# fabrii4/AutoEncoder-FFT

Measured on AMD Instinct MI355X. Metric: frames/s fwd+bwd (FFT mode, 512x512, 4 layers), higher is better.
Workload: dtype f32; 1 GPU; cfg3-P2: 512x512x3 frames, 4 pairs 3->8->16->32->64, 5x5, pool 2/layer, FFT mode, fwd + 1 loop-body iteration per pair (operator form); every step produces reconstructions, batch-mean gradients, updated weights and the per-pair post-update MSE partial sums -- the sums themselves are formed by the next step's gradient launch (no per-step MSE read-back inside the timed loop); frames_per_gpu=32, global_batch=32, parallelism=dp1

## Files before the change

### autoencoder-fft_amd/csrc/internal.h

```cpp
#pragma once
#include <hip/hip_runtime.h>
#include <stddef.h>
#include <stdint.h>

namespace aefft {

extern unsigned dev_flags;
inline bool flag(unsigned f) { return (dev_flags & f) != 0; }

constexpr int TW_N = 4096;
hipError_t upload_twiddles(hipStream_t st);
bool fft_size_supported(int n);

hipError_t launch_r2c(const void* in, float2* out, float2* mid, long planes, int Nx, int Ny,
                      int Nxs, int Nys, hipStream_t st, hipEvent_t done = nullptr , bool in_u8 = false);
constexpr int OPIN_COLS = 4;
constexpr int OPMSE_PACKED_STEPS = 16;
constexpr int CH_MAXSTEPS = 40;
constexpr int CH_VMAX = 128;
struct OpIn { const float2* A; const float2* Xf; int D0, Nx0, Ny0; };
hipError_t launch_c2r(const float2* in, void* out, float2* mid, long planes, int Nxi, int Nyi,
                      int Nx, int Ny, float scale, hipStream_t st, const OpIn* opin = nullptr, bool out_u8 = false);
size_t fft_mid_elems(long planes, int Nx, int Wc);
bool fft_size_supported_any(int n);
size_t fft_any_ws_elems(long planes, int Nx, int Ny);
hipError_t launch_r2c_any(const float* in, float2* out, float2* w1, float2* w2, long planes, int Nx, int Ny, hipStream_t st);
hipError_t launch_c2r_any(const float2* in, float* out, float2* w1, float2* w2, long planes, int Nx, int Ny, float scale, hipStream_t st);
bool fft_size_mixed(int n);
bool fft_size_smooth(int n);
hipError_t fft_mixed_prepare(int n);
hipError_t launch_mix_r2c_rows(const void* in, float2* mid, long npairs, int Ny, int Wc, hipStream_t st, bool in_u8);
hipError_t launch_mix_fwd_cols(const float2* mid, float2* out, long planes, int Nx, int Wc, int Nxs, hipStream_t st, hipEvent_t done);
hipError_t launch_mix_inv_cols(const float2* in, float2* mid, long planes, int Nx, int Wc, int Nxi, hipStream_t st,
                               const OpIn* opin = nullptr );
hipError_t launch_mix_c2r_rows(const float2* mid, void* out, long npairs, int Ny, int Wc, float scale, hipStream_t st, bool out_u8 = false);

struct Contract {
    const float2* A; long a_r, a_k;
    const float2* A2;
    const float2* B; long b_k, b_c;
    float2* Out;     long o_r, o_c;
    int R, C, K;
    long P;
    bool conjA, conjB;
    float preDivB;
    float postDiv;
    const float* bias; float biasScale;
    bool biasAfterFirst;
    int biasColP1;
    int upNx, upNy, upNxs, upNys;
    float2* Out2; int dnNx, dnNy, dnNxs, dnNys;
// ... 183 lines not shown
```

### autoencoder-fft_amd/csrc/opform_kernels.hip

```cpp
#include "../../include/aefft.h"
#include "internal.h"
#include <hip/hip_ext.h>
#include "device_util.h"
#include "opform_device.h"
#include <algorithm>
#include <type_traits>

namespace aefft {

__device__ __forceinline__ float2 cmul(float2 a, float2 b) { return make_float2(a.x * b.x - a.y * b.y, a.x * b.y + a.y * b.x); }
__device__ __forceinline__ float2 cmulc(float2 a, float2 b) { return make_float2(a.x * b.x + a.y * b.y, a.y * b.x - a.x * b.y); }
__device__ __forceinline__ void cfma2(float2& acc, float2 a, float2 b) { acc.x = fmaf(a.x, b.x, acc.x); acc.x = fmaf(-a.y, b.y, acc.x); acc.y = fmaf(a.x, b.y, acc.y); acc.y = fmaf(a.y, b.x, acc.y); }
__device__ __forceinline__ void cfmac(float2& acc, float2 a, float2 b) { acc.x = fmaf(a.x, b.x, acc.x); acc.x = fmaf(a.y, b.y, acc.x); acc.y = fmaf(a.y, b.x, acc.y); acc.y = fmaf(-a.x, b.y, acc.y); }
__device__ __forceinline__ float2 ld8(const float2* base, unsigned e) { return *reinterpret_cast<const float2*>(reinterpret_cast<const char*>(base) + e * 8u); }
__device__ __forceinline__ void st8(float2* base, unsigned e, float2 v) { *reinterpret_cast<float2*>(reinterpret_cast<char*>(base) + e * 8u) = v; }

template <typename MG> __device__ __forceinline__ float quad_centred(const float2 (&r)[OPC], MG Mget)
{
    float2 r3 = r[OPC - 1];
#pragma unroll
    for (int j = 0; j < OPC - 1; ++j) cfma2(r3, r[j], Mget(j * OPC + OPC - 1));
    float part = Mget(OPC * OPC - 1).x * (r3.x * r3.x + r3.y * r3.y);
#pragma unroll
    for (int k = 0; k < OPC - 1; ++k) {
// ... 631 lines not shown
#pragma unroll
    for (int off = 32; off > 0; off >>= 1) part += __shfl_down(part, off, 64);
    float* red = reinterpret_cast<float*>(Ts + (size_t)DM * OPC * BT);
    if ((threadIdx.x & 63) == 0) red[threadIdx.x >> 6] = part;
    __syncthreads();
    if (threadIdx.x == 0) {
        const float tot = (red[0] + red[1]) + (red[2] + red[3]);
        if (tot != 0.f) atomicAdd(q.slots + (blockIdx.x % MSE_SLOTS) * MSE_SLOT_STRIDE, tot * q.scale);
    }
}

#ifndef AEFFT_X_CHAINPIPE
#define AEFFT_X_CHAINPIPE 1
#endif
#ifndef AEFFT_X_CH_DEPTH
#define AEFFT_X_CH_DEPTH 4
#endif
#ifndef AEFFT_X_CH_PK
#define AEFFT_X_CH_PK 1
#endif
__device__ __forceinline__ void cfma_pk(float2& acc, float2 a, float2 b)
{
#if AEFFT_X_CH_PK
    typedef float v2f __attribute__((ext_vector_type(2)));
    v2f r = {acc.x, acc.y};
    const v2f av = {a.x, a.y}, bv = {b.x, b.y};
    asm("v_pk_fma_f32 %0, %1, %2, %0 op_sel:[0,0,0] op_sel_hi:[0,1,1]" : "+v"(r) : "v"(av), "v"(bv));
    asm("v_pk_fma_f32 %0, %1, %2, %0 op_sel:[1,1,0] op_sel_hi:[1,0,1] neg_lo:[0,1,0]" : "+v"(r) : "v"(av), "v"(bv));
    acc = make_float2(r.x, r.y);
#else
    cfma2(acc, a, b);
#endif
}
constexpr int CH_NE = 4, CH_DEPTH = AEFFT_X_CH_DEPTH, CH_NB = CH_DEPTH + 1, CH_KSH_MAX = 4, CH_BLOCK = 12;
template <int N> __device__ __forceinline__ float dpp_row_shl(float v)
{
    return __builtin_bit_cast(float, __builtin_amdgcn_update_dpp(0, __builtin_bit_cast(int, v), 0x100 + N, 0xf, 0xf, true));
}
struct ChainSrc {
    const ChainArgs& g;
    __device__ __forceinline__ unsigned off(int i) const { return g.st_off[i]; }
    __device__ __forceinline__ unsigned desc(int i) const { return g.st_desc[i]; }
    __device__ __forceinline__ const float* bias(unsigned lv, bool enc) const { return enc ? g.lv[lv].b : g.lv[lv].p; }
    __device__ __forceinline__ float NN(unsigned lv) const { return (float)g.lv[lv].Nx * (float)g.lv[lv].Ny; }
    __device__ __forceinline__ float2* out(unsigned lv) const { return g.lv[lv].O; }
    __device__ __forceinline__ unsigned Pc() const { return (unsigned)g.Pc; }
};
template <class SRC>
__device__ __forceinline__ void chain_step_load(const SRC& g, const float2* __restrict__ rec, const int i, float2 (&w)[CH_NE], float& bv)
{
    const unsigned d = g.desc(i), off = g.off(i) & 0xffffffu;
    const unsigned R = d & 255u, K = (d >> 8) & 255u, k0 = (d >> 16) & 127u, ksh = (d >> 23) & 7u;
    const unsigned tid = threadIdx.x;
    const unsigned r = min(tid >> ksh, R - 1u), ks = tid & ((1u << ksh) - 1u);
    const unsigned row = off + r * K, e0 = row + k0 + ks, elast = row + K - 1u;
#pragma unroll
    for (int u = 0; u < CH_NE; ++u) w[u] = ld8(rec, min(e0 + ((unsigned)u << ksh), elast));
    bv = g.bias(d >> 29, (d >> 28) & 1u)[r];
}
template <bool DUAL, class SRC>
__device__ __forceinline__ void chain_step_compute(const SRC& g, const int i, const float2 (&w)[CH_NE], const float bv, float2 (&acc)[OPC], float2 (&acc2)[OPC],
                                                   float2* const Wl, const int t)
{
    static_assert(OPC == 4, "two 16-byte LDS accesses per row of V");
    const unsigned d = g.desc(i), par = g.off(i) >> 31;
    const bool dual = DUAL && ((g.off(i) >> 30) & 1u);
    const unsigned R = d & 255u, K = (d >> 8) & 255u, k0 = (d >> 16) & 127u, ksh = (d >> 23) & 7u;
// ... 84 lines not shown
            }
        }
    }
    __syncthreads();
#if defined(AEFFT_X_WGTIME) && AEFFT_X_WGTIME
    if (threadIdx.x == 0) reinterpret_cast<unsigned long long*>(Wl + 5 * CH_VMAX * OPC + 4 + OPC * OPC)[(enc ? lv : 7 - lv) & 7] = wall_clock64();
#endif
}
template <int I, bool DUAL, class SRC>
__device__ __forceinline__ void chain_steps(const SRC& g, const float2* __restrict__ rec, const int base, const int nb, float2 (&w)[CH_NB][CH_NE], float (&bv)[CH_NB],
                                            float2 (&acc)[OPC], float2 (&acc2)[OPC], float2* const Wl, const int t)
{
    if constexpr (I < CH_BLOCK) {
        if (I >= nb) return;
        chain_step_load(g, rec, base + min(I + CH_DEPTH, nb - 1), w[(I + CH_DEPTH) % CH_NB], bv[(I + CH_DEPTH) % CH_NB]);
        chain_step_compute<DUAL>(g, base + I, w[I % CH_NB], bv[I % CH_NB], acc, acc2, Wl, t);
        chain_steps<I + 1, DUAL, SRC>(g, rec, base, nb, w, bv, acc, acc2, Wl, t);
    }
}
template <bool DUAL, class SRC, class INIT>
__device__ __forceinline__ void chain_run_steps(const SRC& g, const float2* __restrict__ rec, const int n, float2* const Wl, const int t, INIT init)
{
    float2 w[CH_NB][CH_NE];
    float bv[CH_NB];
    float2 acc[OPC], acc2[OPC];
    for (int base = 0; base < n; base += CH_BLOCK) {
        const int nb = min(n - base, CH_BLOCK);
#pragma unroll
        for (int j = 0; j < CH_DEPTH; ++j) chain_step_load(g, rec, base + min(j, nb - 1), w[j], bv[j]);
        if (base == 0) { init(); __syncthreads(); }
        chain_steps<0, DUAL, SRC>(g, rec, base, nb, w, bv, acc, acc2, Wl, t);
    }
}
static bool chain_add_stage(unsigned* st_off, unsigned* st_desc, int* n, int cap, int R, int K, unsigned off, int par, bool enc, int lvl)
{
    int ksh = 0;
    while (ksh < CH_KSH_MAX && (2 << ksh) * R <= 256 && (1 << ksh) < K) ++ksh;
    const int kc = CH_NE << ksh;
    for (int k0 = 0; k0 < K; k0 += kc) {
        if (*n >= cap || off >= (1u << 24) || k0 > 127 || R > 255 || K > 255) return false;
        st_off[*n] = off | ((unsigned)(par & 1) << 31);
        st_desc[*n] = (unsigned)R | ((unsigned)K << 8) | ((unsigned)k0 << 16) | ((unsigned)ksh << 23) | ((k0 + kc >= K ? 1u : 0u) << 26) |
                      ((k0 == 0 ? 1u : 0u) << 27) | ((enc ? 1u : 0u) << 28) | ((unsigned)lvl << 29);
        ++*n;
    }
    return true;
}

constexpr size_t OPMSE_PACKED_LDS = sizeof(float2) * (3 * CH_VMAX * OPC + 2 + OPC * OPC) + 128;
struct PackedMseSrc {
    const OpMseGroup& g; const OpMsePair& q;
    __device__ __forceinline__ unsigned off(int i) const { return g.pst_off[i]; }
    __device__ __forceinline__ unsigned desc(int i) const { return g.pst_desc[i]; }
    __device__ __forceinline__ const float* bias(unsigned, bool enc) const { return enc ? q.b : q.p; }
    __device__ __forceinline__ float NN(unsigned) const { return (float)q.Nx * (float)q.Ny; }
    __device__ __forceinline__ float2* out(unsigned) const { return nullptr; }
    __device__ __forceinline__ unsigned Pc() const { return 0u; }
};
__device__ __forceinline__ void opmse_packed(const OpMseGroup& g, int p, long t, float2* sh)
{
    float2 *Va = sh + 2 * CH_VMAX * OPC;
    float* redp = reinterpret_cast<float*>(sh + 3 * CH_VMAX * OPC);
    const OpMsePair q = g.q[p];
    const int dD = q.dD, dM = q.dM;
    const float2* rec = g.Wp + t * g.E;
    const float2* Vc;
    float2* Ms = sh + 3 * CH_VMAX * OPC + 2;
    const long um = map_up(t, q.Nx, q.Ny, g.Nx0, g.Ny0);
    if (g.pst_n > 0) {
        const PackedMseSrc src{g, q};
        chain_run_steps<false>(src, rec, g.pst_n, sh, (int)t, [&]() {
            float2 mv = make_float2(0.f, 0.f);
            if (threadIdx.x < OPC * OPC) mv = g.Mhat[(long)threadIdx.x * g.P0 + um];
            for (int i = threadIdx.x; i < dD * OPC; i += 256) { const int a = i / OPC, k = i - a * OPC; const float2 v = q.A[((long)k * dD + a) * q.P + t]; sh[i] = v; Va[i] = v; }
            if (threadIdx.x < OPC * OPC) Ms[threadIdx.x] = mv;
        });
        Vc = sh;
    } else {
        float2 *Vb = sh, *Vd = sh + CH_VMAX * OPC;
        if (threadIdx.x < OPC * OPC) Ms[threadIdx.x] = g.Mhat[(long)threadIdx.x * g.P0 + um];
        for (int i = threadIdx.x; i < dD * OPC; i += 256) { const int a = i / OPC, k = i - a * OPC; Va[i] = q.A[((long)k * dD + a) * q.P + t]; }
        const float NN = (float)q.Nx * (float)q.Ny;
        __syncthreads();
        chain_stage_rec(rec + g.offC, Va, Vb, dM, dD, 1.0f / (float)dM, q.b, NN, t == 0, nullptr, 0, 0);
        __syncthreads();
        chain_stage_rec(rec + g.offF, Vb, Vd, dD, dM, 1.0f / (float)dD, q.p, NN, t == 0, nullptr, 0, 0);
        __syncthreads();
        Vc = Vd;
    }
    float part = 0.f;
    if ((int)threadIdx.x < dD) {
        const int a = threadIdx.x;
        float2 r[OPC];
#pragma unroll
        for (int k = 0; k < OPC; ++k) { const float2 av = Va[a * OPC + k], fv = Vc[a * OPC + k]; r[k] = make_float2(av.x - fv.x, av.y - fv.y); }
        part = quad_centred(r, [&](int e) { return Ms[e]; });
        const int nyr = q.Ny / 2 + 1;
        const int j = (int)((unsigned)t % (unsigned)nyr);
        part *= (j > 0 && j < nyr - 1) ? 2.f : 1.f;
    }
#pragma unroll
    for (int off = 32; off > 0; off >>= 1) part += __shfl_down(part, off, 64);
    if ((threadIdx.x & 63) == 0) redp[threadIdx.x >> 6] = part;
    __syncthreads();
    if (threadIdx.x == 0) {
        const float tot = (redp[0] + redp[1]) + (redp[2] + redp[3]);
        if (tot != 0.f) atomicAdd(q.slots + (blockIdx.x % MSE_SLOTS) * MSE_SLOT_STRIDE, tot * q.scale);
    }
}

template <bool LEAN>
__device__ __forceinline__ void opmse_dispatch(const OpMseGroup& g, float2* sh)
{
    const int blk = (int)blockIdx.x - g.base;
    int p = g.n - 1;
#pragma unroll
    for (int i = 6; i >= 0; --i) if (i < g.n - 1 && blk >= g.start[i] - g.base) p = i;
    if (p == g.n - 1 && g.Wp) { opmse_packed(g, p, (long)blockIdx.x - g.start[p], sh); return; }
    if (LEAN || g.q[p].G) { opmse_gbody(g, p, sh); return; }
    if constexpr (!LEAN) {
        const int bt = g.bt[p];
        if (bt == 32) opmse_small_body<8>(g, p, sh);
        else if (bt == 16) opmse_body<16>(g, p, sh);
        else if (bt == 8) opmse_body<8>(g, p, sh);
        else opmse_body<4>(g, p, sh);
    }
}

static hipError_t opmse_geometry(OpMseGroup& g, int base, long* nblocks, size_t* lds_out, bool fused = false )
{
    if (g.n < 1 || g.n > 8) return hipErrorInvalidValue;
    long total = base;
    size_t lds = 0;
    g.base = base;
    for (int i = g.n - 1; i >= 0; --i) {
        const OpMsePair& q = g.q[i];
        int bt = 16;
        while (bt > 4 && ((q.P + bt - 1) / bt < 128 || (size_t)OPC * (q.dD + q.dM) * bt * sizeof(float2) > 48 * 1024)) bt >>= 1;
        size_t need = (size_t)OPC * (q.dD + q.dM) * bt * sizeof(float2) + 64 + (size_t)256 * OPC * sizeof(float2) + (size_t)OPC * OPC * bt * sizeof(float2);
        const bool pk = i == g.n - 1 && g.Wp && q.dD <= CH_VMAX && q.dM <= CH_VMAX;
        if (pk) {
            need = OPMSE_PACKED_LDS;
            int n = 0;
            const bool fits = chain_add_stage(g.pst_off, g.pst_desc, &n, OPMSE_PACKED_STEPS, q.dM, q.dD, (unsigned)g.offC, 0, true, 0) &&
                              chain_add_stage(g.pst_off, g.pst_desc, &n, OPMSE_PACKED_STEPS, q.dD, q.dM, (unsigned)g.offF, 1, false, 0);
            g.pst_n = fits && AEFFT_X_CHAINPIPE ? n : 0;
        }
        else if (q.G) {
            if ((double)q.dD * q.dD * q.P * 8.0 >= 4294967296.0) return hipErrorInvalidValue;
            bt = msgrad_bt(q.dD, q.P);
            need = sizeof(float2) * ((size_t)OPC * q.dD * bt + (size_t)OPC * OPC * bt) + 64;
        } else if (q.dM == 8 && q.dD <= 4 && !flag(AEFFT_F_NOFAST)) { bt = 32; need = (size_t)OPC * (4 + 8) * 32 * sizeof(float2) + 64; }
        if (i == g.n - 1 && !pk) g.Wp = nullptr;
        if (need > 150 * 1024) return hipErrorInvalidValue;
        g.bt[i] = bt;
        lds = std::max(lds, need);
        g.start[i] = (int)total;
        total += pk ? (fused ? 0 : q.P) : (q.P + bt - 1) / bt;
    }
    if (total >= (1L << 31)) return hipErrorInvalidValue;
    g.start[g.n] = (int)total;
    *nblocks = total - base; *lds_out = lds;
    return hipSuccess;
}

}

namespace aefft {

template <int NK> __global__ __launch_bounds__(256) void kspec_packed_kernel(const PackArgs g)
{
    extern __shared__ float2 pk_lds[];
    kspec_packed_body<NK>(g, PackPhasePow2{}, blockIdx.x, blockIdx.y, pk_lds);
}
template <int NK> __global__ __launch_bounds__(256) void kspec_packed_mod_kernel(const PackArgs g, const PackTabs t)
{
    extern __shared__ float2 pk_lds[];
    kspec_packed_body<NK>(g, PackPhaseMod{t}, blockIdx.x, blockIdx.y, pk_lds);
}

void pack_blocks(PackArgs& g)
{
    int nb = 0;
    for (int i = 0; i < g.nseg; ++i)
        for (int l0 = 0; l0 < g.seg[i].n && nb < 128; l0 += 256) { g.blk_seg[nb] = (unsigned char)i; g.blk_start[nb] = l0; ++nb; }
    g.nblk = nb;
}

hipError_t launch_kspec_packed(PackArgs& g, hipStream_t st)
{
    if (g.nseg < 1 || g.nseg > 16 || g.L < 1 || g.L > 8 || g.E < 1 || (g.Nk != 3 && g.Nk != 5)) return hipErrorInvalidValue;
    pack_blocks(g);
    const dim3 grid((unsigned)g.nblk, (unsigned)pack_yblocks(g));
    if (pack_mod(g)) {
        PackTabs t{};
        const hipError_t e = pack_tabs(g, t);
        if (e != hipSuccess) return e;
        if (g.Nk == 3) kspec_packed_mod_kernel<3><<<grid, 256, kspec_packed_lds(3), st>>>(g, t);
        else kspec_packed_mod_kernel<5><<<grid, 256, kspec_packed_lds(5), st>>>(g, t);
        return hipGetLastError();
    }
    if (g.Nk == 3) kspec_packed_kernel<3><<<grid, 256, kspec_packed_lds(3), st>>>(g);
    else kspec_packed_kernel<5><<<grid, 256, kspec_packed_lds(5), st>>>(g);
    return hipGetLastError();
}

template <bool DUAL>
__device__ __forceinline__ void chain_item_run(const ChainArgs& g, const int t, float2* Wl, const OpMseGroup* mse)
{
    const ChainSrc src{g};
    constexpr int VS = CH_VMAX * OPC;
    float2* Ms = Wl + 5 * VS;
    chain_run_steps<DUAL>(src, g.Wp + (long)t * g.E, g.st_n, Wl, t, [&]() {
        float2 mv = make_float2(0.f, 0.f);
        if (DUAL) {
            const OpMsePair& q = mse->q[mse->n - 1];
            if (threadIdx.x < OPC * OPC) mv = mse->Mhat[(long)threadIdx.x * mse->P0 + map_up(t, q.Nx, q.Ny, mse->Nx0, mse->Ny0)];
            const int dD = q.dD;
            for (int i = threadIdx.x; i < dD * OPC; i += 256) { const int a = i / OPC, k = i - a * OPC; Wl[2 * VS + i] = q.A[((long)k * dD + a) * q.P + t]; }
        }
        for (int i = threadIdx.x; i < VS; i += 256) { const int k = i / OPC, c = i - k * OPC; Wl[i] = make_float2((k == c && c < OPC - 1) ? 1.f : 0.f, 0.f); }
        if (DUAL && threadIdx.x < OPC * OPC) Ms[threadIdx.x] = mv;
    });
    if (DUAL) {
        const OpMsePair& q = mse->q[mse->n - 1];
        const float2 *Va = Wl + 2 * VS, *Vc = Wl + 4 * VS;
        float* redp = reinterpret_cast<float*>(Ms + OPC * OPC);
        float part = 0.f;
        if ((int)threadIdx.x < q.dD) {
            const int a = threadIdx.x;
            float2 r[OPC];
#pragma unroll
            for (int k = 0; k < OPC; ++k) { const float2 av = Va[a * OPC + k], fv = Vc[a * OPC + k]; r[k] = make_float2(av.x - fv.x, av.y - fv.y); }
            part = quad_centred(r, [&](int e) { return Ms[e]; });
            const int nyr = q.Ny / 2 + 1;
            const int j = (int)((unsigned)t % (unsigned)nyr);
            part *= (j > 0 && j < nyr - 1) ? 2.f : 1.f;
        }
#pragma unroll
        for (int off = 32; off > 0; off >>= 1) part += __shfl_down(part, off, 64);
        if ((threadIdx.x & 63) == 0) redp[threadIdx.x >> 6] = part;
        __syncthreads();
        if (threadIdx.x == 0) {
            const float tot = (redp[0] + redp[1]) + (redp[2] + redp[3]);
            if (tot != 0.f) atomicAdd(q.slots + (blockIdx.x % MSE_SLOTS) * MSE_SLOT_STRIDE, tot * q.scale);
        }
    }
#if defined(AEFFT_X_WGTIME) && AEFFT_X_WGTIME
    if (threadIdx.x == 0 && g_wgtime && blockIdx.x < WGT_MAX)
        for (int k = 0; k < 8; ++k) g_wgtime[(size_t)5 * WGT_MAX * 2 + ((size_t)4 * WGT_MAX + blockIdx.x) * 8 + k] = reinterpret_cast<unsigned long long*>(Wl + 5 * CH_VMAX * OPC + 4 + OPC * OPC)[k];
#endif
}

#if defined(AEFFT_X_WGTIME) && AEFFT_X_WGTIME
constexpr int CH_ITEM_VECS = 5;
#else
constexpr int CH_ITEM_VECS = 2;
#endif
constexpr int CH_BT = 8;
template <bool FUSE>
__device__ __forceinline__ void chain_body(const ChainArgs& g, const int bx, float2* Wl, const OpMseGroup* mse = nullptr)
{
    const int tid = threadIdx.x;
    const int L = g.L;
    if (AEFFT_X_CHAINPIPE && (long)bx < g.Pc && g.st_n > 0) { chain_item_run<FUSE>(g, bx, Wl, mse); return; }
    if ((long)bx < g.Pc) {
        const int t = bx;
        const bool dc = t == 0;
        const float2* rec = g.Wp + (long)t * g.E;
        for (int i = tid; i < CH_VMAX * OPC; i += 256) { const int k = i / OPC, c = i - k * OPC; Wl[i] = make_float2((k == c && c < OPC - 1) ? 1.f : 0.f, 0.f); }
        int off = 0, si = 0;
        auto run = [&](int R, int K, float scale, const float* bias, float NN, float2* out) {
            __syncthreads();
            AEFFT_WGSTAMP(4, si & 7);
            chain_stage_rec(rec + off, Wl + (si & 1) * (CH_VMAX * OPC), Wl + ((si + 1) & 1) * (CH_VMAX * OPC), R, K, scale, bias, NN, dc, out, g.Pc, t);
            off += (R * K + 1) & ~1; ++si;
        };
        for (int j = 1; j < L; ++j) { const ChainLevel& w = g.lv[j - 1]; run(w.dM, w.dD, 1.0f / (float)w.dM, w.b, (float)w.Nx * (float)w.Ny, nullptr); }
        { const ChainLevel& w = g.lv[L - 1]; run(w.dM, w.dD, 1.0f / (float)w.dM, w.b, (float)w.Nx * (float)w.Ny, nullptr); }
        for (int j = L - 1; j >= 0; --j) { const ChainLevel& v = g.lv[j]; run(v.dD, v.dM, 1.0f / (float)v.dD, v.p, (float)v.Nx * (float)v.Ny, v.O); }
        return;
    }
    int j = 1;
#pragma unroll
    for (int i = 2; i < 8; ++i) if (i < L && bx >= g.tile_start[i]) j = i;
    const int bt = g.tile_bt[j], RT = 256 / bt;
    const int bl = tid & (bt - 1), ry = tid / bt;
    const ChainLevel lj = g.lv[j];
    const long s0 = (long)(bx - g.tile_start[j]) * bt;
    const long s = min(s0 + bl, lj.P - 1);
    const bool ok = s0 + bl < lj.P;
    for (int i = tid; i < OPC * OPC * bt; i += 256) { const int c = (i / bt) % OPC, k = i / (bt * OPC); Wl[i] = make_float2((k == c && c < OPC - 1) ? 1.f : 0.f, 0.f); }
#pragma unroll 1
    for (int i = 1; i <= j; ++i) {
        const ChainLevel& w = g.lv[i - 1];
        const long sbi = i == j ? s : map_up(s, lj.Nx, lj.Ny, g.lv[i].Nx, g.lv[i].Ny);
        const long sbm = map_up(s, lj.Nx, lj.Ny, w.Nx, w.Ny);
        const int R = w.dM, K = w.dD;
// ... 5 lines not shown
            float2 acc[OPC];
#pragma unroll
            for (int c = 0; c < OPC; ++c) acc[c] = make_float2(0.f, 0.f);
            const long pst = w.Cc ? g.lv[i].P : w.P;
            const float2* Wp = (w.Cc ? w.Cc + sbi : w.C + sbm) + (long)r * K * pst;
            auto grp = [&](int k0, auto NU) {
                constexpr int U = decltype(NU)::value;
                float2 wv[U];
#pragma unroll
                for (int u = 0; u < U; ++u) wv[u] = Wp[(long)(k0 + u) * pst];
#pragma unroll
                for (int u = 0; u < U; ++u)
#pragma unroll
                    for (int c = 0; c < OPC; ++c) cfma2(acc[c], wv[u], Vin[((k0 + u) * OPC + c) * bt + bl]);
            };
            int k0 = 0;
            for (; k0 + 16 <= K; k0 += 16) grp(k0, std::integral_constant<int, 16>{});
            if (k0 + 8 <= K) { grp(k0, std::integral_constant<int, 8>{}); k0 += 8; }
            if (k0 + 4 <= K) { grp(k0, std::integral_constant<int, 4>{}); k0 += 4; }
            if (k0 + 2 <= K) { grp(k0, std::integral_constant<int, 2>{}); k0 += 2; }
            if (k0 < K) grp(k0, std::integral_constant<int, 1>{});
#pragma unroll
            for (int c = 0; c < OPC; ++c) { acc[c].x *= scale; acc[c].y *= scale; }
            if (sbi == 0) acc[OPC - 1].x += w.b[r] * NN;
#pragma unroll
            for (int c = 0; c < OPC; ++c) {
                Vout[(r * OPC + c) * bt + bl] = acc[c];
                if (i == j && ok) lj.A[((long)c * R + r) * lj.P + s] = acc[c];
            }
        }
    }
}

__global__ __launch_bounds__(256) void chain_kernel(const ChainArgs g)
{
    extern __shared__ float2 Wl[];
    chain_body<false>(g, blockIdx.x, Wl);
}

static hipError_t chain_geometry(ChainArgs& g, long* nblocks, size_t* lds_out, bool* fuse = nullptr, unsigned offC = 0, unsigned offF = 0)
{
    if (g.L < 1 || g.L > 8 || !g.Wp || g.Pc < 1) return hipErrorInvalidValue;
    for (int l = 0; l < g.L; ++l) {
        if (g.lv[l].dD > CH_VMAX || g.lv[l].dM > CH_VMAX) return hipErrorInvalidValue;
        if (l + 1 < g.L && (size_t)2 * g.lv[l].dM * OPC * CH_BT > CH_WL) return hipErrorInvalidValue;
    }
    {
        int n = 0; unsigned off = 0;
        bool fits = true, offs_ok = true;
        int dual_lo = 0, dual_hi = 0;
        for (int si = 0; si < 2 * g.L && fits; ++si) {
            const bool enc = si < g.L;
            const int l = enc ? si : 2 * g.L - 1 - si;
            const int R = enc ? g.lv[l].dM : g.lv[l].dD, K = enc ? g.lv[l].dD : g.lv[l].dM;
            if (si == g.L - 1) { dual_lo = n; offs_ok = offs_ok && off == offC; }
            if (si == g.L) offs_ok = offs_ok && off == offF;
            fits = chain_add_stage(g.st_off, g.st_desc, &n, CH_MAXSTEPS, R, K, off, si & 1, enc, l);
            if (si == g.L) dual_hi = n;
            off += (unsigned)((R * K + 1) & ~1);
        }
        g.st_n = fits ? n : 0;
        if (fuse) {
            *fuse = *fuse && fits && offs_ok && AEFFT_X_CHAINPIPE;
            if (*fuse) for (int i = dual_lo; i < dual_hi; ++i) g.st_off[i] |= 1u << 30;
        }
        if ((double)OPC * CH_VMAX * (double)g.Pc * sizeof(float2) >= 4294967296.0) return hipErrorInvalidValue;
    }
    long total = g.Pc;
    int vt = OPC * OPC * 32;
    for (int j = 1; j < g.L; ++j) {
        int rj = OPC;
        for (int l = 0; l < j; ++l) rj = std::max(rj, g.lv[l].dM);
        int bt = 32;
        while (bt > CH_BT && bt * rj > 256) bt >>= 1;
        g.tile_bt[j] = bt;
        vt = std::max(vt, rj * OPC * bt);
        g.tile_start[j] = (int)total; total += (g.lv[j].P + bt - 1) / bt;
    }
    g.tile_start[g.L] = (int)total;
    if (total >= (1L << 31)) return hipErrorInvalidValue;
    g.vt_elems = vt;
    *nblocks = total;
    *lds_out = std::max(sizeof(float2) * 2 * g.vt_elems, sizeof(float2) * ((fuse && *fuse ? 5 : CH_ITEM_VECS) * (size_t)CH_VMAX * OPC + OPC * OPC + 4) + 256 );
    return hipSuccess;
}

hipError_t launch_chain(ChainArgs& g, hipStream_t st, hipEvent_t done)
{
    long total; size_t lds;
    const hipError_t eg = chain_geometry(g, &total, &lds);
    if (eg != hipSuccess) return eg;
    if (done) hipExtLaunchKernelGGL(chain_kernel, dim3((unsigned)total), dim3(256), lds, st, nullptr, done, 0, g);
    else chain_kernel<<<dim3((unsigned)total), 256, lds, st>>>(g);
    return hipGetLastError();
}

#ifndef AEFFT_X_TAIL_W
#define AEFFT_X_TAIL_W 6
#endif
#ifndef AEFFT_X_TAIL_WF
#define AEFFT_X_TAIL_WF 5
#endif
template <bool LEAN, bool FUSE>
__global__ __launch_bounds__(256, LEAN ? (FUSE ? AEFFT_X_TAIL_WF : AEFFT_X_TAIL_W) : 4) void tail_kernel(const OpMseGroup g, const ChainArgs ch, const UpdateGroup ug, const int nchain, const int nupd_start)
{
    AEFFT_WGTIME(4);
    extern __shared__ float2 sh[];
    if ((int)blockIdx.x < nchain) { chain_body<FUSE>(ch, blockIdx.x, sh, &g); return; }
    if ((int)blockIdx.x >= nupd_start) {
        const int blk = blockIdx.x - nupd_start;
        int p = 0;
#pragma unroll
        for (int i = 1; i < 8; ++i) if (i < ug.n && blk >= ug.start[i]) p = i;
        update_weights_part(ug.a[p], blk - ug.start[p]);
        return;
    }
    opmse_dispatch<LEAN>(g, sh);
}

static UpdateGroup g_tail_ug_none{};
static ChainArgs g_tail_chain_none{};
hipError_t launch_opmse_group(OpMseGroup& g, hipStream_t st, ChainArgs* chain, const UpdateGroup* weights_upd)
{
    long nchain = 0, nmse = 0;
    size_t lds_c = 0, lds_m = 0;
#ifndef AEFFT_X_FUSEMSE
#define AEFFT_X_FUSEMSE 1
#endif
    bool fuse = AEFFT_X_FUSEMSE && chain && g.Wp && chain->Wp == g.Wp && chain->E == g.E && chain->Pc == g.q[g.n - 1].P &&
                g.q[g.n - 1].dD <= CH_VMAX && g.q[g.n - 1].dM <= CH_VMAX && g.q[g.n - 1].dD <= 256;
    if (chain) { const hipError_t e = chain_geometry(*chain, &nchain, &lds_c, &fuse, (unsigned)g.offC, (unsigned)g.offF); if (e != hipSuccess) return e; }
    { const hipError_t e = opmse_geometry(g, (int)nchain, &nmse, &lds_m, false); if (e != hipSuccess) return e; }
    if (fuse && nchain + nmse < 4 * 1536 && !flag(AEFFT_F_CHAINMSE)) {
        fuse = false;
        for (int i = 0; i < chain->st_n; ++i) chain->st_off[i] &= ~(1u << 30);
        const hipError_t e = chain_geometry(*chain, &nchain, &lds_c); if (e != hipSuccess) return e;
    }
    if (fuse) {
        const hipError_t e = opmse_geometry(g, (int)nchain, &nmse, &lds_m, true); if (e != hipSuccess) return e;
        if (!g.Wp) return hipErrorInvalidValue;
    }
    int nupd = 0;
    UpdateGroup ug = g_tail_ug_none;
    if (weights_upd && weights_upd->n > 0) {
        ug = *weights_upd;
        for (int i = 0; i < ug.n; ++i) { ug.start[i] = nupd; nupd += (ug.a[i].dM * ug.a[i].dD * ug.a[i].Nk * ug.a[i].Nl + 255) / 256; }
        ug.start[ug.n] = nupd;
    }
    const size_t lds = std::max(lds_c, lds_m);
#ifndef AEFFT_X_LEANTAIL
#define AEFFT_X_LEANTAIL 1
#endif
    bool lean = AEFFT_X_LEANTAIL != 0;
    for (int i = 0; i < g.n && lean; ++i) lean = g.q[i].G != nullptr || (i == g.n - 1 && g.Wp != nullptr);
    const long total = nchain + nmse + nupd;
    if (total >= (1L << 31)) return hipErrorInvalidValue;
    auto go = [&](auto LEANT, auto FUSET) -> hipError_t {
        constexpr bool LN = decltype(LEANT)::value, FS = decltype(FUSET)::value;
        if (lds > 64 * 1024) {
            const hipError_t e = hipFuncSetAttribute(reinterpret_cast<const void*>(tail_kernel<LN, FS>), hipFuncAttributeMaxDynamicSharedMemorySize, (int)lds);
            if (e != hipSuccess) return e;
        }
        tail_kernel<LN, FS><<<dim3((unsigned)total), 256, lds, st>>>(g, chain ? *chain : g_tail_chain_none, ug, (int)nchain, (int)(nchain + nmse));
        return hipGetLastError();
    };
    if (lean) return fuse ? go(std::true_type{}, std::true_type{}) : go(std::true_type{}, std::false_type{});
    return fuse ? go(std::false_type{}, std::true_type{}) : go(std::false_type{}, std::false_type{});
}

}

#if defined(AEFFT_X_WGTIME) && AEFFT_X_WGTIME
extern "C" int aefft_debug_wgtime_opform(void* p) { return aefft::wgtime_set_tu(p); }
#endif
```

Before: 222,400 frames/s.

## Specialize chain step pipeline at compile time for known layer plans

Result: no change. 223,500 frames/s (median of 5 runs) (+0.5%).

```diff
diff --git a/autoencoder-fft_amd/csrc/chain_plan.h b/autoencoder-fft_amd/csrc/chain_plan.h
--- /dev/null
+++ b/autoencoder-fft_amd/csrc/chain_plan.h
@@ -0,0 +1,91 @@
+#pragma once
+
+namespace aefft {
+
+constexpr int OPMSE_PACKED_STEPS = 16;
+constexpr int CH_MAXSTEPS = 40;
+constexpr int CH_NE = 4, CH_KSH_MAX = 4;
+
+constexpr unsigned CH_OFF_DUAL = 1u << 30;
+constexpr bool chain_add_stage(unsigned* st_off, unsigned* st_desc, int* n, int cap, int R, int K, unsigned off, int par, bool enc, int lvl)
+{
+    int ksh = 0;
+    while (ksh < CH_KSH_MAX && (2 << ksh) * R <= 256 && (1 << ksh) < K) ++ksh;
+    const int kc = CH_NE << ksh;
+    for (int k0 = 0; k0 < K; k0 += kc) {
+        if (*n >= cap || off >= (1u << 24) || k0 > 127 || R > 255 || K > 255) return false;
+        st_off[*n] = off | ((unsigned)(par & 1) << 31);
+        st_desc[*n] = (unsigned)R | ((unsigned)K << 8) | ((unsigned)k0 << 16) | ((unsigned)ksh << 23) | ((k0 + kc >= K ? 1u : 0u) << 26) |
+                      ((k0 == 0 ? 1u : 0u) << 27) | ((enc ? 1u : 0u) << 28) | ((unsigned)lvl << 29);
+        ++*n;
+    }
+    return true;
+}
+
+constexpr bool chain_list_build(unsigned* st_off, unsigned* st_desc, int* n_out, int L, const int* dD, const int* dM, int* dual_lo, int* dual_hi,
+                                unsigned* recC, unsigned* recF)
+{
+    int n = 0; unsigned off = 0;
+    bool fits = true;
+    for (int si = 0; si < 2 * L && fits; ++si) {
+        const bool enc = si < L;
+        const int l = enc ? si : 2 * L - 1 - si;
+        const int R = enc ? dM[l] : dD[l], K = enc ? dD[l] : dM[l];
+        if (si == L - 1) { *dual_lo = n; *recC = off; }
+        if (si == L) *recF = off;
+        fits = chain_add_stage(st_off, st_desc, &n, CH_MAXSTEPS, R, K, off, si & 1, enc, l);
+        if (si == L) *dual_hi = n;
+        off += (unsigned)((R * K + 1) & ~1);
+    }
+    *n_out = n;
+    return fits;
+}
+constexpr bool chain_list_build_mse(unsigned* st_off, unsigned* st_desc, int* n_out, int dD, int dM, unsigned offC, unsigned offF)
+{
+    int n = 0;
+    const bool fits = chain_add_stage(st_off, st_desc, &n, OPMSE_PACKED_STEPS, dM, dD, offC, 0, true, 0) &&
+                      chain_add_stage(st_off, st_desc, &n, OPMSE_PACKED_STEPS, dD, dM, offF, 1, false, 0);
+    *n_out = n;
+    return fits;
+}
+
+struct ChainPlan {
+    unsigned off[CH_MAXSTEPS] = {}, desc[CH_MAXSTEPS] = {}; int n = 0;
+    unsigned moff[OPMSE_PACKED_STEPS] = {}, mdesc[OPMSE_PACKED_STEPS] = {}; int mn = 0;
+};
+constexpr int CH_PLAN_MIN = 3, CH_PLAN_MAX = 5;
+constexpr ChainPlan chain_plan_make(int PL)
+{
+    ChainPlan p;
+    int dD[8] = {}, dM[8] = {};
+    for (int l = 0; l < PL; ++l) { dM[l] = 8 << l; dD[l] = l ? dM[l - 1] : 3; }
+    int lo = 0, hi = 0; unsigned recC = 0, recF = 0;
+    if (!chain_list_build(p.off, p.desc, &p.n, PL, dD, dM, &lo, &hi, &recC, &recF)) p.n = 0;
+    for (int i = lo; i < hi && i < p.n; ++i) p.off[i] |= CH_OFF_DUAL;
+    if (!chain_list_build_mse(p.moff, p.mdesc, &p.mn, dD[PL - 1], dM[PL - 1], recC, recF)) p.mn = 0;
+    return p;
+}
+template <int PL> inline constexpr ChainPlan chain_plan_v = chain_plan_make(PL);
+
+constexpr bool chain_list_same(const unsigned* off, const unsigned* desc, int n, const unsigned* poff, const unsigned* pdesc, int pn)
+{
+    if (n != pn || n < 1) return false;
+    for (int i = 0; i < n; ++i) if (((off[i] ^ poff[i]) & ~CH_OFF_DUAL) != 0 || desc[i] != pdesc[i]) return false;
+    return true;
+}
+constexpr int chain_plan_of(const unsigned* off, const unsigned* desc, int n)
+{
+    if (chain_list_same(off, desc, n, chain_plan_v<3>.off, chain_plan_v<3>.desc, chain_plan_v<3>.n)) return 3;
+    if (chain_list_same(off, desc, n, chain_plan_v<4>.off, chain_plan_v<4>.desc, chain_plan_v<4>.n)) return 4;
+    if (chain_list_same(off, desc, n, chain_plan_v<5>.off, chain_plan_v<5>.desc, chain_plan_v<5>.n)) return 5;
+    return 0;
+}
+constexpr int chain_plan_of_mse(const unsigned* off, const unsigned* desc, int n)
+{
+    if (chain_list_same(off, desc, n, chain_plan_v<3>.moff, chain_plan_v<3>.mdesc, chain_plan_v<3>.mn)) return 3;
+    if (chain_list_same(off, desc, n, chain_plan_v<4>.moff, chain_plan_v<4>.mdesc, chain_plan_v<4>.mn)) return 4;
+    if (chain_list_same(off, desc, n, chain_plan_v<5>.moff, chain_plan_v<5>.mdesc, chain_plan_v<5>.mn)) return 5;
+    return 0;
+}
+
+}
diff --git a/autoencoder-fft_amd/csrc/internal.h b/autoencoder-fft_amd/csrc/internal.h
--- a/autoencoder-fft_amd/csrc/internal.h
+++ b/autoencoder-fft_amd/csrc/internal.h
@@ -2,6 +2,7 @@
 #include <hip/hip_runtime.h>
 #include <stddef.h>
 #include <stdint.h>
+#include "chain_plan.h"
 
 namespace aefft {
 
@@ -15,8 +16,6 @@
 hipError_t launch_r2c(const void* in, float2* out, float2* mid, long planes, int Nx, int Ny,
                       int Nxs, int Nys, hipStream_t st, hipEvent_t done = nullptr , bool in_u8 = false);
 constexpr int OPIN_COLS = 4;
-constexpr int OPMSE_PACKED_STEPS = 16;
-constexpr int CH_MAXSTEPS = 40;
 constexpr int CH_VMAX = 128;
 struct OpIn { const float2* A; const float2* Xf; int D0, Nx0, Ny0; };
 hipError_t launch_c2r(const float2* in, void* out, float2* mid, long planes, int Nxi, int Nyi,
diff --git a/autoencoder-fft_amd/csrc/opform_kernels.hip b/autoencoder-fft_amd/csrc/opform_kernels.hip
--- a/autoencoder-fft_amd/csrc/opform_kernels.hip
+++ b/autoencoder-fft_amd/csrc/opform_kernels.hip
@@ -687,7 +687,7 @@
     cfma2(acc, a, b);
 #endif
 }
-constexpr int CH_NE = 4, CH_DEPTH = AEFFT_X_CH_DEPTH, CH_NB = CH_DEPTH + 1, CH_KSH_MAX = 4, CH_BLOCK = 12;
+constexpr int CH_DEPTH = AEFFT_X_CH_DEPTH, CH_NB = CH_DEPTH + 1, CH_BLOCK = 12;
 template <int N> __device__ __forceinline__ float dpp_row_shl(float v)
 {
     return __builtin_bit_cast(float, __builtin_amdgcn_update_dpp(0, __builtin_bit_cast(int, v), 0x100 + N, 0xf, 0xf, true));
@@ -838,19 +838,140 @@
         chain_steps<0, DUAL, SRC>(g, rec, base, nb, w, bv, acc, acc2, Wl, t);
     }
 }
-static bool chain_add_stage(unsigned* st_off, unsigned* st_desc, int* n, int cap, int R, int K, unsigned off, int par, bool enc, int lvl)
-{
-    int ksh = 0;
-    while (ksh < CH_KSH_MAX && (2 << ksh) * R <= 256 && (1 << ksh) < K) ++ksh;
-    const int kc = CH_NE << ksh;
-    for (int k0 = 0; k0 < K; k0 += kc) {
-        if (*n >= cap || off >= (1u << 24) || k0 > 127 || R > 255 || K > 255) return false;
-        st_off[*n] = off | ((unsigned)(par & 1) << 31);
-        st_desc[*n] = (unsigned)R | ((unsigned)K << 8) | ((unsigned)k0 << 16) | ((unsigned)ksh << 23) | ((k0 + kc >= K ? 1u : 0u) << 26) |
-                      ((k0 == 0 ? 1u : 0u) << 27) | ((enc ? 1u : 0u) << 28) | ((unsigned)lvl << 29);
-        ++*n;
-    }
-    return true;
+
+template <int PL, bool MSE> struct ChainPlanSteps {
+    static constexpr int n = MSE ? chain_plan_v<PL>.mn : chain_plan_v<PL>.n;
+    static constexpr unsigned off(int i) { return MSE ? chain_plan_v<PL>.moff[i] : chain_plan_v<PL>.off[i]; }
+    static constexpr unsigned desc(int i) { return MSE ? chain_plan_v<PL>.mdesc[i] : chain_plan_v<PL>.desc[i]; }
+};
+template <class PS, int I, class SRC>
+__device__ __forceinline__ void chain_xstep_load(const SRC& g, const float2* __restrict__ rec, float2 (&w)[CH_NE], float& bv)
+{
+    constexpr unsigned d = PS::desc(I), off = PS::off(I) & 0xffffffu;
+    constexpr unsigned R = d & 255u, K = (d >> 8) & 255u, k0 = (d >> 16) & 127u, ksh = (d >> 23) & 7u, KS = 1u << ksh;
+    const unsigned tid = threadIdx.x;
+    const unsigned rr = tid >> ksh, ks = tid & (KS - 1u);
+    const unsigned r = (256u >> ksh) > R ? min(rr, R - 1u) : rr;
+    const unsigned row = off + r * K, e0 = row + k0 + ks;
+#pragma unroll
+    for (unsigned u = 0; u < (unsigned)CH_NE; ++u) {
+        const unsigned kb = k0 + (u << ksh);
+        if (kb >= K) continue;
+        w[u] = ld8(rec, kb + KS <= K ? e0 + (u << ksh) : min(e0 + (u << ksh), row + K - 1u));
+    }
+    if constexpr ((d >> 26) & 1u) bv = g.bias(d >> 29, (d >> 28) & 1u)[r];
+}
+template <class PS, int I, bool DUALK, class SRC>
+__device__ __forceinline__ void chain_xstep_compute(const SRC& g, const float2 (&w)[CH_NE], const float bv, float2 (&acc)[OPC], float2 (&acc2)[OPC], float2* const Wl, const int t)
+{
+    static_assert(OPC == 4, "two 16-byte LDS accesses per row of V");
+    constexpr unsigned d = PS::desc(I), par = PS::off(I) >> 31;
+    constexpr bool dual = DUALK && ((PS::off(I) >> 30) & 1u);
+    constexpr unsigned R = d & 255u, K = (d >> 8) & 255u, k0 = (d >> 16) & 127u, ksh = (d >> 23) & 7u, KS = 1u << ksh, lv = d >> 29;
+    constexpr bool enc = (d >> 28) & 1u;
+    const unsigned tid = threadIdx.x;
+    const unsigned rr = tid >> ksh, ks = tid & (KS - 1u);
+    if constexpr ((d >> 27) & 1u) {
+#pragma unroll
+        for (int c = 0; c < OPC; ++c) { acc[c] = make_float2(0.f, 0.f); if (DUALK) acc2[c] = make_float2(0.f, 0.f); }
+    }
+    const float2* Vin = Wl + par * (CH_VMAX * OPC);
+    const float2* Vin2 = Wl + (enc ? 2 : 3) * (CH_VMAX * OPC);
+#pragma unroll
+    for (unsigned u = 0; u < (unsigned)CH_NE; ++u) {
+        const unsigned kb = k0 + (u << ksh);
+        if (kb >= K) continue;
+        const bool full = kb + KS <= K;
+        const unsigned k = kb + ks;
+        const float2 wv = (full || k < K) ? w[u] : make_float2(0.f, 0.f);
+        const unsigned kk = (full ? k : min(k, K - 1u)) * OPC;
+        {
+            const float4* vp = reinterpret_cast<const float4*>(Vin + kk);
+            const float4 va = vp[0], vb = vp[1];
+            cfma_pk(acc[0], wv, make_float2(va.x, va.y)); cfma_pk(acc[1], wv, make_float2(va.z, va.w));
+            cfma_pk(acc[2], wv, make_float2(vb.x, vb.y)); cfma_pk(acc[3], wv, make_float2(vb.z, vb.w));
+        }
+        if constexpr (dual) {
+            const float4* vp = reinterpret_cast<const float4*>(Vin2 + kk);
+            const float4 va = vp[0], vb = vp[1];
+            cfma_pk(acc2[0], wv, make_float2(va.x, va.y)); cfma_pk(acc2[1], wv, make_float2(va.z, va.w));
+            cfma_pk(acc2[2], wv, make_float2(vb.x, vb.y)); cfma_pk(acc2[3], wv, make_float2(vb.z, vb.w));
+        }
+    }
+    if constexpr ((d >> 26) & 1u) {
+        auto rung = [&](auto NT) {
+            constexpr int N = decltype(NT)::value;
+#pragma unroll
+            for (int c = 0; c < OPC; ++c) { acc[c].x += dpp_row_shl<N>(acc[c].x); acc[c].y += dpp_row_shl<N>(acc[c].y); }
+            if constexpr (dual) {
+#pragma unroll
+                for (int c = 0; c < OPC; ++c) { acc2[c].x += dpp_row_shl<N>(acc2[c].x); acc2[c].y += dpp_row_shl<N>(acc2[c].y); }
+            }
+        };
+        if constexpr (ksh > 0) rung(std::integral_constant<int, 1>{});
+        if constexpr (ksh > 1) rung(std::integral_constant<int, 2>{});
+        if constexpr (ksh > 2) rung(std::integral_constant<int, 4>{});
+        if constexpr (ksh > 3) rung(std::integral_constant<int, 8>{});
+        if (((256u >> ksh) <= R || rr < R) && ks == 0) {
+            constexpr float scale = 1.0f / (float)R;
+#pragma unroll
+            for (int c = 0; c < OPC; ++c) { acc[c].x *= scale; acc[c].y *= scale; }
+            if (t == 0) acc[OPC - 1].x += bv * g.NN(lv);
+            if constexpr (dual) {
+#pragma unroll
+                for (int c = 0; c < OPC; ++c) { acc2[c].x *= scale; acc2[c].y *= scale; }
+                if (t == 0) acc2[OPC - 1].x += bv * g.NN(lv);
+                float4* v2 = reinterpret_cast<float4*>(Wl + (enc ? 3 : 4) * (CH_VMAX * OPC) + rr * OPC);
+                v2[0] = make_float4(acc2[0].x, acc2[0].y, acc2[1].x, acc2[1].y); v2[1] = make_float4(acc2[2].x, acc2[2].y, acc2[3].x, acc2[3].y);
+            }
+            const float4 o0 = make_float4(acc[0].x, acc[0].y, acc[1].x, acc[1].y), o1 = make_float4(acc[2].x, acc[2].y, acc[3].x, acc[3].y);
+            float4* vo = reinterpret_cast<float4*>(Wl + (par ^ 1u) * (CH_VMAX * OPC) + rr * OPC);
+            vo[0] = o0; vo[1] = o1;
+            if constexpr (!enc) {
+                float2* O = g.out(lv);
+                if (O) {
+                    const unsigned Pc = g.Pc();
+#pragma unroll
+                    for (int c = 0; c < OPC; ++c) st8(O, ((unsigned)c * R + rr) * Pc + (unsigned)t, acc[c]);
+                }
+            }
+        }
+        __syncthreads();
+#if defined(AEFFT_X_WGTIME) && AEFFT_X_WGTIME
+        if (threadIdx.x == 0) reinterpret_cast<unsigned long long*>(Wl + 5 * CH_VMAX * OPC + 4 + OPC * OPC)[(enc ? lv : 7 - lv) & 7] = wall_clock64();
+#endif
+    }
+}
+template <class PS, int J, class SRC>
+__device__ __forceinline__ void chain_xsteps_fill(const SRC& g, const float2* __restrict__ rec, float2 (&w)[CH_NB][CH_NE], float (&bv)[CH_NB])
+{
+    if constexpr (J < CH_DEPTH && J < PS::n) {
+        chain_xstep_load<PS, J>(g, rec, w[J], bv[J]);
+        __builtin_amdgcn_sched_barrier(0);
+        chain_xsteps_fill<PS, J + 1>(g, rec, w, bv);
+    }
+}
+template <class PS, int I, bool DUALK, class SRC>
+__device__ __forceinline__ void chain_xsteps(const SRC& g, const float2* __restrict__ rec, float2 (&w)[CH_NB][CH_NE], float (&bv)[CH_NB],
+                                             float2 (&acc)[OPC], float2 (&acc2)[OPC], float2* const Wl, const int t)
+{
+    if constexpr (I < PS::n) {
+        if constexpr (I + CH_DEPTH < PS::n) chain_xstep_load<PS, I + CH_DEPTH>(g, rec, w[(I + CH_DEPTH) % CH_NB], bv[(I + CH_DEPTH) % CH_NB]);
+        __builtin_amdgcn_sched_barrier(0);
+        chain_xstep_compute<PS, I, DUALK>(g, w[I % CH_NB], bv[I % CH_NB], acc, acc2, Wl, t);
+        __builtin_amdgcn_sched_barrier(0);
+        chain_xsteps<PS, I + 1, DUALK>(g, rec, w, bv, acc, acc2, Wl, t);
+    }
+}
+template <class PS, bool DUALK, class SRC, class INIT>
+__device__ __forceinline__ void chain_run_xsteps(const SRC& g, const float2* __restrict__ rec, float2* const Wl, const int t, INIT init)
+{
+    float2 w[CH_NB][CH_NE];
+    float bv[CH_NB];
+    float2 acc[OPC], acc2[OPC];
+    chain_xsteps_fill<PS, 0>(g, rec, w, bv);
+    init(); __syncthreads();
+    chain_xsteps<PS, 0, DUALK>(g, rec, w, bv, acc, acc2, Wl, t);
 }
 
 constexpr size_t OPMSE_PACKED_LDS = sizeof(float2) * (3 * CH_VMAX * OPC + 2 + OPC * OPC) + 128;
@@ -863,6 +984,7 @@
     __device__ __forceinline__ float2* out(unsigned) const { return nullptr; }
     __device__ __forceinline__ unsigned Pc() const { return 0u; }
 };
+template <int PL>
 __device__ __forceinline__ void opmse_packed(const OpMseGroup& g, int p, long t, float2* sh)
 {
     float2 *Va = sh + 2 * CH_VMAX * OPC;
@@ -873,16 +995,18 @@
     const float2* Vc;
     float2* Ms = sh + 3 * CH_VMAX * OPC + 2;
     const long um = map_up(t, q.Nx, q.Ny, g.Nx0, g.Ny0);
-    if (g.pst_n > 0) {
+    if (PL || g.pst_n > 0) {
         const PackedMseSrc src{g, q};
-        chain_run_steps<false>(src, rec, g.pst_n, sh, (int)t, [&]() {
+        auto init = [&]() {
             float2 mv = make_float2(0.f, 0.f);
             if (threadIdx.x < OPC * OPC) mv = g.Mhat[(long)threadIdx.x * g.P0 + um];
             for (int i = threadIdx.x; i < dD * OPC; i += 256) { const int a = i / OPC, k = i - a * OPC; const float2 v = q.A[((long)k * dD + a) * q.P + t]; sh[i] = v; Va[i] = v; }
             if (threadIdx.x < OPC * OPC) Ms[threadIdx.x] = mv;
-        });
+        };
+        if constexpr (PL != 0) chain_run_xsteps<ChainPlanSteps<PL, true>, false>(src, rec, sh, (int)t, init);
+        else chain_run_steps<false>(src, rec, g.pst_n, sh, (int)t, init);
         Vc = sh;
-    } else {
+    } else if constexpr (PL == 0) {
         float2 *Vb = sh, *Vd = sh + CH_VMAX * OPC;
         if (threadIdx.x < OPC * OPC) Ms[threadIdx.x] = g.Mhat[(long)threadIdx.x * g.P0 + um];
         for (int i = threadIdx.x; i < dD * OPC; i += 256) { const int a = i / OPC, k = i - a * OPC; Va[i] = q.A[((long)k * dD + a) * q.P + t]; }
@@ -893,7 +1017,7 @@
         chain_stage_rec(rec + g.offF, Vb, Vd, dD, dM, 1.0f / (float)dD, q.p, NN, t == 0, nullptr, 0, 0);
         __syncthreads();
         Vc = Vd;
-    }
+    } else Vc = sh;
     float part = 0.f;
     if ((int)threadIdx.x < dD) {
         const int a = threadIdx.x;
@@ -915,14 +1039,14 @@
     }
 }
 
-template <bool LEAN>
+template <bool LEAN, int PL>
 __device__ __forceinline__ void opmse_dispatch(const OpMseGroup& g, float2* sh)
 {
     const int blk = (int)blockIdx.x - g.base;
     int p = g.n - 1;
 #pragma unroll
     for (int i = 6; i >= 0; --i) if (i < g.n - 1 && blk >= g.start[i] - g.base) p = i;
-    if (p == g.n - 1 && g.Wp) { opmse_packed(g, p, (long)blockIdx.x - g.start[p], sh); return; }
+    if (p == g.n - 1 && g.Wp) { opmse_packed<PL>(g, p, (long)blockIdx.x - g.start[p], sh); return; }
     if (LEAN || g.q[p].G) { opmse_gbody(g, p, sh); return; }
     if constexpr (!LEAN) {
         const int bt = g.bt[p];
@@ -948,8 +1072,7 @@
         if (pk) {
             need = OPMSE_PACKED_LDS;
             int n = 0;
-            const bool fits = chain_add_stage(g.pst_off, g.pst_desc, &n, OPMSE_PACKED_STEPS, q.dM, q.dD, (unsigned)g.offC, 0, true, 0) &&
-                              chain_add_stage(g.pst_off, g.pst_desc, &n, OPMSE_PACKED_STEPS, q.dD, q.dM, (unsigned)g.offF, 1, false, 0);
+            const bool fits = chain_list_build_mse(g.pst_off, g.pst_desc, &n, q.dD, q.dM, (unsigned)g.offC, (unsigned)g.offF);
             g.pst_n = fits && AEFFT_X_CHAINPIPE ? n : 0;
         }
         else if (q.G) {
@@ -1011,13 +1134,13 @@
     return hipGetLastError();
 }
 
-template <bool DUAL>
+template <bool DUAL, int PL>
 __device__ __forceinline__ void chain_item_run(const ChainArgs& g, const int t, float2* Wl, const OpMseGroup* mse)
 {
     const ChainSrc src{g};
     constexpr int VS = CH_VMAX * OPC;
     float2* Ms = Wl + 5 * VS;
-    chain_run_steps<DUAL>(src, g.Wp + (long)t * g.E, g.st_n, Wl, t, [&]() {
+    auto init = [&]() {
         float2 mv = make_float2(0.f, 0.f);
         if (DUAL) {
             const OpMsePair& q = mse->q[mse->n - 1];
@@ -1027,7 +1150,9 @@
         }
         for (int i = threadIdx.x; i < VS; i += 256) { const int k = i / OPC, c = i - k * OPC; Wl[i] = make_float2((k == c && c < OPC - 1) ? 1.f : 0.f, 0.f); }
         if (DUAL && threadIdx.x < OPC * OPC) Ms[threadIdx.x] = mv;
-    });
+    };
+    if constexpr (PL != 0) chain_run_xsteps<ChainPlanSteps<PL, false>, DUAL>(src, g.Wp + (long)t * g.E, Wl, t, init);
+    else chain_run_steps<DUAL>(src, g.Wp + (long)t * g.E, g.st_n, Wl, t, init);
     if (DUAL) {
         const OpMsePair& q = mse->q[mse->n - 1];
         const float2 *Va = Wl + 2 * VS, *Vc = Wl + 4 * VS;
@@ -1064,12 +1189,12 @@
 constexpr int CH_ITEM_VECS = 2;
 #endif
 constexpr int CH_BT = 8;
-template <bool FUSE>
+template <bool FUSE, int PL = 0>
 __device__ __forceinline__ void chain_body(const ChainArgs& g, const int bx, float2* Wl, const OpMseGroup* mse = nullptr)
 {
     const int tid = threadIdx.x;
     const int L = g.L;
-    if (AEFFT_X_CHAINPIPE && (long)bx < g.Pc && g.st_n > 0) { chain_item_run<FUSE>(g, bx, Wl, mse); return; }
+    if (AEFFT_X_CHAINPIPE && (long)bx < g.Pc && g.st_n > 0) { chain_item_run<FUSE, PL>(g, bx, Wl, mse); return; }
     if ((long)bx < g.Pc) {
         const int t = bx;
         const bool dc = t == 0;
@@ -1141,11 +1266,13 @@
     }
 }
 
+template <int PL>
 __global__ __launch_bounds__(256) void chain_kernel(const ChainArgs g)
 {
     extern __shared__ float2 Wl[];
-    chain_body<false>(g, blockIdx.x, Wl);
-}
+    chain_body<false, PL>(g, blockIdx.x, Wl);
+}
+static int chain_exact_plan(const ChainArgs& g) { return g.st_n > 0 && AEFFT_X_CHAINPIPE && !flag(AEFFT_F_NOFAST) ? chain_plan_of(g.st_off, g.st_desc, g.st_n) : 0; }
 
 static hipError_t chain_geometry(ChainArgs& g, long* nblocks, size_t* lds_out, bool* fuse = nullptr, unsigned offC = 0, unsigned offF = 0)
 {
@@ -1155,23 +1282,16 @@
         if (l + 1 < g.L && (size_t)2 * g.lv[l].dM * OPC * CH_BT > CH_WL) return hipErrorInvalidValue;
     }
     {
-        int n = 0; unsigned off = 0;
-        bool fits = true, offs_ok = true;
+        int n = 0, dD[8], dM[8];
+        for (int l = 0; l < g.L; ++l) { dD[l] = g.lv[l].dD; dM[l] = g.lv[l].dM; }
         int dual_lo = 0, dual_hi = 0;
-        for (int si = 0; si < 2 * g.L && fits; ++si) {
-            const bool enc = si < g.L;
-            const int l = enc ? si : 2 * g.L - 1 - si;
-            const int R = enc ? g.lv[l].dM : g.lv[l].dD, K = enc ? g.lv[l].dD : g.lv[l].dM;
-            if (si == g.L - 1) { dual_lo = n; offs_ok = offs_ok && off == offC; }
-            if (si == g.L) offs_ok = offs_ok && off == offF;
-            fits = chain_add_stage(g.st_off, g.st_desc, &n, CH_MAXSTEPS, R, K, off, si & 1, enc, l);
-            if (si == g.L) dual_hi = n;
-            off += (unsigned)((R * K + 1) & ~1);
-        }
+        unsigned recC = 0, recF = 0;
+        const bool fits = chain_list_build(g.st_off, g.st_desc, &n, g.L, dD, dM, &dual_lo, &dual_hi, &recC, &recF);
+        const bool offs_ok = fits && recC == offC && recF == offF;
         g.st_n = fits ? n : 0;
         if (fuse) {
             *fuse = *fuse && fits && offs_ok && AEFFT_X_CHAINPIPE;
-            if (*fuse) for (int i = dual_lo; i < dual_hi; ++i) g.st_off[i] |= 1u << 30;
+            if (*fuse) for (int i = dual_lo; i < dual_hi; ++i) g.st_off[i] |= CH_OFF_DUAL;
         }
         if ((double)OPC * CH_VMAX * (double)g.Pc * sizeof(float2) >= 4294967296.0) return hipErrorInvalidValue;
     }
@@ -1199,9 +1319,18 @@
     long total; size_t lds;
     const hipError_t eg = chain_geometry(g, &total, &lds);
     if (eg != hipSuccess) return eg;
-    if (done) hipExtLaunchKernelGGL(chain_kernel, dim3((unsigned)total), dim3(256), lds, st, nullptr, done, 0, g);
-    else chain_kernel<<<dim3((unsigned)total), 256, lds, st>>>(g);
-    return hipGetLastError();
+    auto go = [&](auto PLT) -> hipError_t {
+        constexpr int PL = decltype(PLT)::value;
+        if (done) hipExtLaunchKernelGGL(chain_kernel<PL>, dim3((unsigned)total), dim3(256), lds, st, nullptr, done, 0, g);
+        else chain_kernel<PL><<<dim3((unsigned)total), 256, lds, st>>>(g);
+        return hipGetLastError();
+    };
+    switch (chain_exact_plan(g)) {
+        case 3: return go(std::integral_constant<int, 3>{});
+        case 4: return go(std::integral_constant<int, 4>{});
+        case 5: return go(std::integral_constant<int, 5>{});
+        default: return go(std::integral_constant<int, 0>{});
+    }
 }
 
 #ifndef AEFFT_X_TAIL_W
@@ -1210,12 +1339,12 @@
 #ifndef AEFFT_X_TAIL_WF
 #define AEFFT_X_TAIL_WF 5
 #endif
-template <bool LEAN, bool FUSE>
+template <bool LEAN, bool FUSE, int PL>
 __global__ __launch_bounds__(256, LEAN ? (FUSE ? AEFFT_X_TAIL_WF : AEFFT_X_TAIL_W) : 4) void tail_kernel(const OpMseGroup g, const ChainArgs ch, const UpdateGroup ug, const int nchain, const int nupd_start)
 {
     AEFFT_WGTIME(4);
     extern __shared__ float2 sh[];
-    if ((int)blockIdx.x < nchain) { chain_body<FUSE>(ch, blockIdx.x, sh, &g); return; }
+    if ((int)blockIdx.x < nchain) { chain_body<FUSE, PL>(ch, blockIdx.x, sh, &g); return; }
     if ((int)blockIdx.x >= nupd_start) {
         const int blk = blockIdx.x - nupd_start;
         int p = 0;
@@ -1224,7 +1353,7 @@
         update_weights_part(ug.a[p], blk - ug.start[p]);
         return;
     }
-    opmse_dispatch<LEAN>(g, sh);
+    opmse_dispatch<LEAN, PL>(g, sh);
 }
 
 static UpdateGroup g_tail_ug_none{};
@@ -1242,7 +1371,7 @@
     { const hipError_t e = opmse_geometry(g, (int)nchain, &nmse, &lds_m, false); if (e != hipSuccess) return e; }
     if (fuse && nchain + nmse < 4 * 1536 && !flag(AEFFT_F_CHAINMSE)) {
         fuse = false;
-        for (int i = 0; i < chain->st_n; ++i) chain->st_off[i] &= ~(1u << 30);
+        for (int i = 0; i < chain->st_n; ++i) chain->st_off[i] &= ~CH_OFF_DUAL;
         const hipError_t e = chain_geometry(*chain, &nchain, &lds_c); if (e != hipSuccess) return e;
     }
     if (fuse) {
@@ -1264,17 +1393,36 @@
     for (int i = 0; i < g.n && lean; ++i) lean = g.q[i].G != nullptr || (i == g.n - 1 && g.Wp != nullptr);
     const long total = nchain + nmse + nupd;
     if (total >= (1L << 31)) return hipErrorInvalidValue;
-    auto go = [&](auto LEANT, auto FUSET) -> hipError_t {
+    auto go = [&](auto LEANT, auto FUSET, auto PLT) -> hipError_t {
         constexpr bool LN = decltype(LEANT)::value, FS = decltype(FUSET)::value;
+        constexpr int PL = decltype(PLT)::value;
         if (lds > 64 * 1024) {
-            const hipError_t e = hipFuncSetAttribute(reinterpret_cast<const void*>(tail_kernel<LN, FS>), hipFuncAttributeMaxDynamicSharedMemorySize, (int)lds);
+            const hipError_t e = hipFuncSetAttribute(reinterpret_cast<const void*>(tail_kernel<LN, FS, PL>), hipFuncAttributeMaxDynamicSharedMemorySize, (int)lds);
             if (e != hipSuccess) return e;
         }
-        tail_kernel<LN, FS><<<dim3((unsigned)total), 256, lds, st>>>(g, chain ? *chain : g_tail_chain_none, ug, (int)nchain, (int)(nchain + nmse));
+        tail_kernel<LN, FS, PL><<<dim3((unsigned)total), 256, lds, st>>>(g, chain ? *chain : g_tail_chain_none, ug, (int)nchain, (int)(nchain + nmse));
         return hipGetLastError();
     };
-    if (lean) return fuse ? go(std::true_type{}, std::true_type{}) : go(std::true_type{}, std::false_type{});
-    return fuse ? go(std::false_type{}, std::true_type{}) : go(std::false_type{}, std::false_type{});
+    int plan = 0;
+    if (lean && !flag(AEFFT_F_NOFAST)) {
+        const bool packed_wgs = g.Wp != nullptr && !fuse;
+        const int pc = chain ? chain_exact_plan(*chain) : 0;
+        const int pm = packed_wgs && g.pst_n > 0 ? chain_plan_of_mse(g.pst_off, g.pst_desc, g.pst_n) : 0;
+        if (chain && packed_wgs) plan = pc == pm ? pc : 0;
+        else if (chain) plan = pc;
+        else if (packed_wgs) plan = pm;
+        if (plan == 5 && !fuse) plan = 0;
+    }
+    const std::true_type T{}; const std::false_type F{};
+    if (lean) {
+        switch (plan) {
+            case 3: return fuse ? go(T, T, std::integral_constant<int, 3>{}) : go(T, F, std::integral_constant<int, 3>{});
+            case 4: return fuse ? go(T, T, std::integral_constant<int, 4>{}) : go(T, F, std::integral_constant<int, 4>{});
+            case 5: return go(T, T, std::integral_constant<int, 5>{});
+            default: return fuse ? go(T, T, std::integral_constant<int, 0>{}) : go(T, F, std::integral_constant<int, 0>{});
+        }
+    }
+    return fuse ? go(F, T, std::integral_constant<int, 0>{}) : go(F, F, std::integral_constant<int, 0>{});
 }
 
 }
```
